# thomasneff/AdaNeRF

Hardware: NVIDIA H100
Metric: frames_per_sec_800x800 (higher is better)
Workload: dtype bf16

## Files before the change

### adanerf_b200/csrc/api.cu

```cuda
#include <cuda_runtime.h>

#include <algorithm>
#include <cmath>
#include <cstdio>
#include <cstdlib>
#include <cstring>
#include <map>
#include <optional>
#include <string>
#include <vector>

#include "../../include/adanerf_b200.h"
#include "export_loader.h"
#include "mlp.cuh"
#include "ptx.cuh"
#include "stages.cuh"

using namespace adn;

namespace {

struct HostTensor {
  std::vector<float> data;
  int64_t rows = 0, cols = 0;
// ... 60 lines not shown
  cudaEvent_t ev[8] = {};
  adn_stats stats{};
  std::string last_error;
};

namespace {

const char* kStatusText[] = {"ok", "invalid argument", "CUDA error", "no usable sm_90 device", "weights not set",
                             "I/O error", "device watchdog tripped"};

adn_status fail(adn_ctx* ctx, adn_status s, const std::string& msg) {
  if (ctx) ctx->last_error = msg;
  return s;
}
adn_status cuda_fail(adn_ctx* ctx, cudaError_t e, const char* where) {
  return fail(ctx, ADN_ERR_CUDA, std::string(where) + ": " + cudaGetErrorString(e));
}
#define ADN_CUDA(ctx, call)                                   \
  do {                                                        \
    cudaError_t e__ = (call);                                 \
    if (e__ != cudaSuccess) return cuda_fail(ctx, e__, #call); \
  } while (0)

adn_status ensure(adn_ctx* ctx, Buf& b, size_t bytes) {
  if (bytes <= b.cap) return ADN_OK;
  ADN_CUDA(ctx, b.release());
  const bool pinned = b.kind == Buf::kPinned;
  const size_t want = pinned ? bytes : bytes + bytes / 8 + 256;
  ADN_CUDA(ctx, pinned ? cudaMallocHost(&b.p, want) : cudaMalloc(&b.p, want));
  b.cap = want;
  return ADN_OK;
}

bool pin_in_place(adn_ctx* ctx, const void* p, size_t bytes) {
  const char* lo = static_cast<const char*>(p);
  for (const adn_ctx::Reg& r : ctx->regs)
    if (lo >= static_cast<const char*>(r.p) && lo + bytes <= static_cast<const char*>(r.p) + r.bytes) return true;
  cudaPointerAttributes attr{};
  if (cudaPointerGetAttributes(&attr, p) == cudaSuccess && attr.type == cudaMemoryTypeHost) return true;
  cudaGetLastError();
  return false;
}

inline uint16_t f2bf(float f) {
  uint32_t u;
  std::memcpy(&u, &f, 4);
  if ((u & 0x7FFFFFFFu) > 0x7F800000u) return uint16_t((u >> 16) | 0x40);
  u += 0x7FFFu + ((u >> 16) & 1u);
  return uint16_t(u >> 16);
}
inline float bf2f(uint16_t h) {
  uint32_t u = uint32_t(h) << 16;
  float f;
  std::memcpy(&f, &u, 4);
  return f;
}

struct Seg {
  int col0, valid;
};

void pack_layer(const float* W, int n_out, int k_in, const std::vector<Seg>& segs, int nsplit, std::vector<uint8_t>& blob) {
  const int n_half = (n_out + 127) / 128;
  for (int nh = 0; nh < n_half; ++nh) {
    for (const Seg& sg : segs) {
      const size_t base = blob.size();
      blob.resize(base + size_t(nsplit) * kBlkBytes, 0);
      for (int n = 0; n < 128; ++n) {
        const int row = nh * 128 + n;
        for (int kk = 0; kk < 64; ++kk) {
          float w = 0.0f;
          if (row < n_out && kk < sg.valid && sg.col0 + kk < k_in) w = W[size_t(row) * k_in + sg.col0 + kk];
          const uint16_t hi = f2bf(w);
          const uint32_t off = sw128_offset(uint32_t(n), uint32_t(kk));
          std::memcpy(&blob[base + off], &hi, 2);
          if (nsplit == 2) {
            const uint16_t lo = f2bf(w - bf2f(hi));
            std::memcpy(&blob[base + kBlkBytes + off], &lo, 2);
          }
        }
      }
    }
  }
}

size_t push_floats(std::vector<float>& f, const float* src, size_t n) {
  while (f.size() % 4) f.push_back(0.0f);
  const size_t off = f.size();
  f.insert(f.end(), src, src + n);
  while (f.size() % 4) f.push_back(0.0f);
  return off;
}

const HostTensor* find(const Net& n, const std::string& name) {
  auto it = n.tensors.find(name);
  return it == n.tensors.end() ? nullptr : &it->second;
}

adn_status upload(adn_ctx* ctx, Net& net, const std::vector<uint8_t>& wblob, const std::vector<float>& fblob) {
  if (fblob.size() > size_t(kSideFloats))
    return fail(ctx, ADN_ERR_INVALID, "network has " + std::to_string(fblob.size()) + " fp32 side parameters (biases and heads), more than " +
                                          std::to_string(kSideFloats) + " fit in shared memory");
  std::memset(net.prog.side, 0, sizeof(net.prog.side));
  std::memcpy(net.prog.side, fblob.data(), fblob.size() * 4);
  adn_status s = ensure(ctx, net.wblob, wblob.size());
  if (s != ADN_OK) return s;
  ADN_CUDA(ctx, cudaMemcpy(net.wblob.p, wblob.data(), wblob.size(), cudaMemcpyHostToDevice));
  return ADN_OK;
}

adn_status build_net0(adn_ctx* ctx) {
  Net& net = ctx->net[0];
  auto bad = [&](const std::string& msg) { return fail(ctx, ADN_ERR_INVALID, "sampling net: " + msg); };
  int D = 0;
  while (find(net, "layers." + std::to_string(D) + ".weight")) ++D;
  if (D < 1 || D > kMaxLayers) return bad("need layers.0.weight .. (1-12 layers)");
  const int nsplit = ctx->mlp0_terms == 3 ? 2 : 1;
  const int width = int(find(net, "layers.0.weight")->rows);
  MlpProgram P{};
  P.n_layers = D;
  std::vector<uint8_t> wblob;
  std::vector<float> fblob;
  int prev = -1;
  for (int l = 0; l < D; ++l) {
    const std::string name = "layers." + std::to_string(l);
    const HostTensor* W = find(net, name + ".weight");
    const HostTensor* B = find(net, name + ".bias");
    if (!B || int64_t(B->data.size()) != W->rows) return bad(name + ".bias is missing or not [" + std::to_string(W->rows) + "]");
    const int n_out = int(W->rows), k_in = int(W->cols);
    const bool last = (l == D - 1);
    if (l == 0) {
      if (k_in < 1 || k_in > 128) return bad(name + ".weight has " + std::to_string(k_in) + " input columns; the input width must be 1-128");
      net.n_in = k_in;
    } else if (k_in != prev) {
      return bad(name + ".weight has " + std::to_string(k_in) + " input columns but layers." + std::to_string(l - 1) + " has " +
                 std::to_string(prev) + " outputs: layer widths must chain (BaseNet skips are not supported)");
    }
    if (!last && n_out != width)
      return bad(name + ".weight has " + std::to_string(n_out) + " outputs; every hidden layer must be as wide as layers.0 (" +
                 std::to_string(width) + ")");
    if (!last && n_out != 128 && n_out != 256)
      return bad(name + ".weight has " + std::to_string(n_out) + " outputs; the hidden width must be 128 or 256");
    if (last && n_out != 128 && n_out != 256)
      return bad(name + ".weight has " + std::to_string(n_out) + " outputs; the output width must be 128 or 256");
    prev = n_out;
    MlpLayer& L = P.layers[l];
    std::vector<Seg> segs;
    if (l == 0) {
      segs = {{0, std::min(64, k_in)}, {64, std::max(0, k_in - 64)}};
    } else {
      for (int c = 0; c < k_in; c += 64) segs.push_back({c, 64});
    }
    L.n_kb = uint8_t(segs.size());
    for (size_t i = 0; i < segs.size(); ++i) {
      L.a_blk[i] = uint8_t(i);
      L.k_cnt[i] = uint8_t(std::max(i == 0 ? 1 : 0, (segs[i].valid + 15) / 16));
    }
    L.n_half = uint8_t(n_out / 128);
    L.flags = last ? uint8_t(LF_FINAL_RAW) : uint8_t(LF_RELU | LF_OUT_ACT);
    L.out_blk0 = 0;
    L.w_off = uint32_t(wblob.size());
    pack_layer(W->data.data(), n_out, k_in, segs, nsplit, wblob);
    L.bias_off = uint32_t(push_floats(fblob, B->data.data(), B->data.size()));
    if (last) {
      net.n_out = n_out;
      P.out_cols = n_out;
    }
  }
  P.in = sampling_tiles(net.n_in, nsplit);
  P.in_nblk0 = P.in.n_blk;
  net.prog = P;
  adn_status s = upload(ctx, net, wblob, fblob);
  if (s != ADN_OK) return s;
  net.depth = D;
  net.width = width;
  net.skip = -1;
  net.ready = true;
  return ADN_OK;
}

adn_status build_net1(adn_ctx* ctx) {
  Net& net = ctx->net[1];
  constexpr int kP = 63, kV = 27;
  auto bad = [&](const std::string& msg) { return fail(ctx, ADN_ERR_INVALID, "shading net: " + msg); };
  auto shape = [](int64_t r, int64_t c) { return "[" + std::to_string(r) + ", " + std::to_string(c) + "]"; };
  const HostTensor* w0 = find(net, "pts_linears.0.weight");
  if (!w0 || w0->cols != kP)
    return bad("pts_linears.0.weight must be [W, 63] (posEnc 10-4)" + (w0 ? ", not " + shape(w0->rows, w0->cols) : std::string(", missing")));
  const int W = int(w0->rows);
  if (W != 128 && W != 256) return bad("pts_linears.0.weight has " + std::to_string(W) + " rows; the width W must be 128 or 256");
  int D = 0;
  while (find(net, "pts_linears." + std::to_string(D) + ".weight")) ++D;
  if (D > kMaxLayers - 2) return bad("pts_linears.0 .. " + std::to_string(D - 1) + ": " + std::to_string(D) + " layers, at most 10 are supported");
  const HostTensor *pw[kMaxLayers], *pb[kMaxLayers];
  int skip = -1;
  for (int i = 0; i < D; ++i) {
    const std::string name = "pts_linears." + std::to_string(i);
    pw[i] = find(net, name + ".weight");
    pb[i] = find(net, name + ".bias");
    if (pw[i]->rows != W) return bad(name + ".weight has " + std::to_string(pw[i]->rows) + " rows; every pts layer must be W = " + std::to_string(W) + " wide");
    if (i > 0 && pw[i]->cols == W + kP) {
      if (skip >= 0)
        return bad(name + ".weight reads cat[pts, h] after the skip at layer " + std::to_string(skip) + "; at most one skip is supported");
      skip = i - 1;
    } else if (i > 0 && pw[i]->cols != W) {
      return bad(name + ".weight has " + std::to_string(pw[i]->cols) + " input columns; expect W = " + std::to_string(W) +
                 " or W + 63 = " + std::to_string(W + kP) + " (a skip)");
    }
    if (!pb[i] || int64_t(pb[i]->data.size()) != W) return bad(name + ".bias is missing or not [" + std::to_string(W) + "]");
  }
  struct Want {
    const char* name;
    int64_t rows, cols;
  };
  const Want want[4] = {{"feature_linear", W, W}, {"alpha_linear", 1, W}, {"views_linears.0", W / 2, W + kV}, {"rgb_linear", 3, W / 2}};
  const HostTensor *hw[4], *hb[4];
  for (int j = 0; j < 4; ++j) {
    const std::string name(want[j].name);
    hw[j] = find(net, name + ".weight");
    hb[j] = find(net, name + ".bias");
    if (!hw[j] || hw[j]->rows != want[j].rows || hw[j]->cols != want[j].cols)
      return bad(name + ".weight must be " + shape(want[j].rows, want[j].cols) + " for W = " + std::to_string(W) + " (posEnc 10-4)" +
                 (hw[j] ? ", not " + shape(hw[j]->rows, hw[j]->cols) : std::string(", missing")));
    if (!hb[j] || int64_t(hb[j]->data.size()) != want[j].rows) return bad(name + ".bias is missing or not [" + std::to_string(want[j].rows) + "]");
  }
  const HostTensor *fw = hw[0], *fb = hb[0], *aw = hw[1], *ab = hb[1], *vw = hw[2], *vb = hb[2], *rw = hw[3], *rb = hb[3];
  net.n_in = kP + kV;
  net.n_out = 4;
  const int nh = W / 64;
  const int load_v = skip >= 0 ? skip + 1 : 0;
  MlpProgram P{};
  P.n_layers = D + 2;
  std::vector<uint8_t> wblob;
  std::vector<float> fblob;
  for (int l = 0; l < D + 2; ++l) {
    MlpLayer& L = P.layers[l];
    std::vector<Seg> segs;
    std::vector<uint8_t> blk;
    auto read_p = [&] { segs.push_back({0, kP}), blk.push_back(0); };
    auto read_hidden = [&](int col0) {
      for (int b = 0; b < nh; ++b) segs.push_back({col0 + 64 * b, 64}), blk.push_back(uint8_t(1 + b));
    };
    const HostTensor *Wt, *B;
    L.out_blk0 = 1;
    L.n_half = uint8_t(W / 128);
    if (l < D) {
      if (l == 0) {
        read_p();
      } else if (l == skip + 1) {
        read_p();
        read_hidden(kP);
      } else {
        read_hidden(0);
      }
      L.flags = LF_RELU | LF_OUT_ACT | (l == D - 1 ? LF_ALPHA_DOT : 0) | (l == load_v ? LF_LOAD_IN1_AFTER : 0);
      Wt = pw[l];
      B = pb[l];
    } else if (l == D) {
      read_hidden(0);
      L.flags = LF_OUT_ACT;
      Wt = fw;
      B = fb;
    } else {
      read_hidden(0);
      segs.push_back({W, kV});
      blk.push_back(0);
      L.flags = LF_RELU | LF_FINAL_RGB | LF_WAIT_IN;
      L.n_half = 1;
      Wt = vw;
      B = vb;
    }
    L.n_kb = uint8_t(segs.size());
    for (size_t i = 0; i < segs.size(); ++i) {
      L.a_blk[i] = blk[i];
      L.k_cnt[i] = uint8_t((segs[i].valid + 15) / 16);
    }
    L.w_off = uint32_t(wblob.size());
    pack_layer(Wt->data.data(), int(Wt->rows), int(Wt->cols), segs, 1, wblob);
    std::vector<float> bias(size_t(L.n_half) * 128, 0.0f);
    std::copy(B->data.begin(), B->data.end(), bias.begin());
    L.bias_off = uint32_t(push_floats(fblob, bias.data(), bias.size()));
  }
  std::vector<float> rgb_w(3 * 128, 0.0f);
  for (int k = 0; k < 3; ++k) std::copy_n(rw->data.data() + size_t(k) * (W / 2), W / 2, rgb_w.data() + k * 128);
  P.alpha_w_off = uint32_t(push_floats(fblob, aw->data.data(), size_t(W)));
  P.alpha_b_off = uint32_t(push_floats(fblob, ab->data.data(), 1));
  P.rgb_w_off = uint32_t(push_floats(fblob, rgb_w.data(), rgb_w.size()));
  P.rgb_b_off = uint32_t(push_floats(fblob, rb->data.data(), 3));
  P.in = shading_tiles();
  P.in_nblk0 = 1;
  P.out_cols = 4;
  net.prog = P;
  adn_status s = upload(ctx, net, wblob, fblob);
  if (s != ADN_OK) return s;
  net.depth = D;
  net.width = W;
  net.skip = skip;
  net.ready = true;
  return ADN_OK;
}

void set_ndc_projection(adn_ctx* ctx, int W, int H, float focal_in) {
  const double focal = focal_in > 0.0f ? double(focal_in) : 0.5 * double(W) / std::tan(0.5 * double(ctx->scene.fov));
  ctx->sc.ndc_cw = float(-1.0 / (double(W) / (2.0 * focal)));
  ctx->sc.ndc_ch = float(-1.0 / (double(H) / (2.0 * focal)));
}

adn_status ensure_dense_lut(adn_ctx* ctx, int K) {
  if (ctx->dense_K == K) return ADN_OK;
  std::vector<float> lut(K);
  const double max_v = double(ctx->scene.depth_range[1]) - double(ctx->scene.depth_range[0]);
  for (int k = 0; k < K; ++k) {
    const float step = 1.0f / float(K);
    const float lin = (k < (K + 1) / 2) ? float(k) * step : 1.0f - float(K - k) * step;
    const float t = lin + float(0.5 / K);
    const float z = ctx->scene.z_near * (1.0f - t) + ctx->scene.z_far * t;
    const float w = float(std::pow(max_v + 1.0, double(z)));
    lut[k] = ctx->scene.use_ndc ? z : (w - 1.0f) + ctx->scene.depth_range[0];
  }
  adn_status s = ensure(ctx, ctx->zlut_dense, sizeof(float) * K);
  if (s != ADN_OK) return s;
  ADN_CUDA(ctx, cudaMemcpy(ctx->zlut_dense.p, lut.data(), sizeof(float) * K, cudaMemcpyHostToDevice));
  ctx->dense_K = K;
  return ADN_OK;
}

PoseDev make_pose(const float* pose, const float* rot) {
  PoseDev p;
  std::memcpy(p.pose, pose, 12);
  std::memcpy(p.rot, rot, 36);
  return p;
}

std::optional<CameraRays> camera_rays(const adn_ctx* ctx, int W, int H, int row0, int rows) {
  if (!ctx || W < 1 || H < 1 || row0 < 0 || rows < 0 || row0 + rows > H) return std::nullopt;
  CameraRays c;
  const double fov = double(ctx->scene.fov);
  const double focal = 0.5 * W / std::tan(0.5 * fov);
  const double x_dist = std::tan(fov / 2) * focal;
  const double y_dist = x_dist * (double(H) / double(W));
  c.x_pp = x_dist / (W / 2.0);
  c.y_pp = y_dist / (H / 2.0);
  c.start_x = -(x_dist - c.x_pp / 2);
  c.start_y = -(y_dist - c.y_pp / 2);
  c.focal = focal;
  c.W = W;
  c.H = H;
  c.row0 = row0;
  return c;
}

int64_t pad128(int64_t n) { return (n + 127) / 128 * 128; }

adn_status run_mlp(adn_ctx* ctx, int id, const uint8_t* tiles, float* out, const long long* rows_dev, long long rows,
                   cudaStream_t st, const EncodeParams* enc = nullptr) {
  Net& n = ctx->net[id];
  const cudaError_t e = launch_mlp(n.prog, n.wblob.as<uint8_t>(), tiles, out, rows_dev, rows, ctx->d_err, ctx->num_sms, st, enc);
  if (e != cudaSuccess) return cuda_fail(ctx, e, id == 0 ? "launch sampling MLP" : "launch shading MLP");
  ctx->stats.kernel_launches++;
  return ADN_OK;
}

struct RenderCall {
  const float* pose;
  const float* rot;
  const float* d_dirs = nullptr;
  std::optional<CameraRays> cam;
  int64_t n_rays;
  float thr;
  int K;
  float* d_rgb = nullptr;
  uint8_t* d_rgba8 = nullptr;
  int32_t* d_nsamples = nullptr;
  float* d_oracle_w = nullptr;
  adn_aux_outputs aux{};
  cudaStream_t st;
  RenderCall(const float* pose_, const float* rot_, int64_t n_rays_, float thr_, int K_, void* stream)
      : pose(pose_), rot(rot_), n_rays(n_rays_), thr(thr_), K(K_), st(static_cast<cudaStream_t>(stream)) {}
};

RenderCall chunk_of(const RenderCall& call, int64_t r0, int64_t chunk) {
  RenderCall c = call;
  c.n_rays = std::min(chunk, call.n_rays - r0);
  if (c.d_dirs) c.d_dirs += 3 * r0;
  if (c.cam) c.cam->row0 += int(r0 / c.cam->W);
  if (c.d_rgb) c.d_rgb += 3 * r0;
  if (c.d_rgba8) c.d_rgba8 += 4 * r0;
  if (c.d_nsamples) c.d_nsamples += r0;
  if (c.d_oracle_w) c.d_oracle_w += 128 * r0;
  for (float** p : {&c.aux.d_weights, &c.aux.d_alpha, &c.aux.d_z_vals})
    if (*p) *p += r0 * c.K;
  for (float** p : {&c.aux.d_depth_map, &c.aux.d_acc_map, &c.aux.d_disp_map, &c.aux.d_depth_est})
    if (*p) *p += r0;
  return c;
}

Stage5Aux stage5_aux(const adn_ctx* ctx, const adn_aux_outputs& a) {
  const adn_scene& sc = ctx->scene;
  return {a.d_weights, a.d_alpha, a.d_z_vals, a.d_depth_map, a.d_acc_map, a.d_disp_map, a.d_depth_est, sc.use_ndc ? 1 : 0,
          sc.depth_range[0], float(std::log(double(sc.depth_range[1]) - double(sc.depth_range[0]) + 1.0))};
}

adn_status run_stages_0_1(adn_ctx* ctx, const RenderCall& c, int64_t w, bool timing) {
  const Net& n0 = ctx->net[0];
  adn_status s = ensure(ctx, ctx->tiles0, size_t(pad128(c.n_rays) / 128) * n0.prog.in.tile_bytes());
  if (s != ADN_OK) return s;
  float* raw0 = c.d_oracle_w ? c.d_oracle_w : ctx->raw0.as<float>() + 128 * w;
  uint8_t* tiles0 = ctx->tiles0.as<uint8_t>();
  if (timing) cudaEventRecord(ctx->ev[0], c.st);
  ADN_CUDA(ctx, launch_stage0(ctx->sc, make_pose(c.pose, c.rot), c.d_dirs, c.cam ? &*c.cam : nullptr, c.n_rays, nullptr,
                              ctx->ray_o.as<float>() + 3 * w, ctx->ray_d.as<float>() + 3 * w, tiles0, n0.prog.in.n_terms, c.st));
  ctx->stats.kernel_launches++;
  if (timing) cudaEventRecord(ctx->ev[1], c.st);
  if ((s = run_mlp(ctx, 0, tiles0, raw0, nullptr, c.n_rays, c.st)) != ADN_OK) return s;
  if (timing) cudaEventRecord(ctx->ev[2], c.st);
  return ADN_OK;
}

adn_status run_stages_2_5(adn_ctx* ctx, const RenderCall& c, int64_t w, const float* d_thr, bool timing) {
  const int64_t n = c.n_rays;
  const int K = c.K;
  const bool dense = (c.thr == 0.0f);
  const int64_t cap = n * K;
  adn_status s;
  if ((s = ensure(ctx, ctx->count, size_t(n) * 4)) != ADN_OK) return s;
  if ((s = ensure(ctx, ctx->offset, size_t(n) * 4)) != ADN_OK) return s;
  if (!dense) {
    if ((s = ensure(ctx, ctx->rayidx, size_t(cap) * 4)) != ADN_OK) return s;
    if ((s = ensure(ctx, ctx->zbuf, size_t(cap) * 4)) != ADN_OK) return s;
// ... 618 lines not shown
```

### adanerf_b200/csrc/mlp.cu

```cuda
#include <cuda_bf16.h>
#include <cuda_runtime.h>

#include "mlp.cuh"
#include "posenc.cuh"
#include "ptx.cuh"
#include "tiles.cuh"

namespace adn {

template <uint8_t V>
struct ConstFlags {
  __device__ constexpr operator uint8_t() const { return V; }
};

template <int NSPLIT>
struct MlpCfg {
  static constexpr int kNB = (NSPLIT == 2) ? 4 : 5;
  static constexpr int kStageBytes = NSPLIT * kBlkBytes;
  static constexpr int kStages = (NSPLIT == 2) ? 2 : 8;
  static constexpr size_t kActBytes = size_t(NSPLIT) * kNB * kBlkBytes;
  static constexpr size_t kSmemBytes =
      kActBytes + size_t(kStages) * kStageBytes + size_t(kSideFloats) * 4 + 2 * kStages * 8 + 1024 ;
};
static_assert(MlpCfg<1>::kSmemBytes <= 232448 && MlpCfg<2>::kSmemBytes <= 232448, "shared memory per block (sm_90)");

template <bool VIEW>
__device__ __forceinline__ void encode_row(const EncodeParams& enc, long long i, long long rows, uint8_t* blk, int row) {
  float f[64];
#pragma unroll
  for (int k = 0; k < 64; ++k) f[k] = 0.0f;
  if (i < rows) {
    long long ray;
    float zw;
    if (enc.ray_idx) {
      ray = enc.ray_idx[i];
      zw = enc.z[i];
    } else {
      ray = i / enc.K;
      zw = enc.zlut_dense[i - ray * enc.K];
    }
    float pos[3], dir[3];
    sample_inputs(enc.sc, false, enc.ray_o, enc.ray_d, ray, zw, pos, dir);
    if (VIEW) posenc3<4>(dir, f);
    else posenc3<10>(pos, f);
  }
#pragma unroll
  for (int ch = 0; ch < 8; ++ch) pack_chunk8(f + ch * 8, uint32_t(row), ch, blk, nullptr);
}

__device__ __forceinline__ void copy_rows(const uint8_t* __restrict__ src, uint32_t dst, int nblk, int wg, int tw) {
  for (int b = 0; b < nblk; ++b) {
    const uint4* s = reinterpret_cast<const uint4*>(src + size_t(b) * kBlkBytes + size_t(wg) * (kBlkBytes / 2));
    const uint32_t d = dst + uint32_t(b) * kBlkBytes + uint32_t(wg) * (kBlkBytes / 2);
    uint4 v[4];
#pragma unroll
    for (int j = 0; j < 4; ++j) v[j] = __ldg(s + tw + 128 * j);
#pragma unroll
    for (int j = 0; j < 4; ++j) st_shared_v4(d + uint32_t(tw + 128 * j) * 16u, v[j].x, v[j].y, v[j].z, v[j].w);
  }
}

template <int NSPLIT, bool ENC>
__global__ void __launch_bounds__(kMlpThreads, 1)
mlp_kernel(const __grid_constant__ MlpProgram prog, const uint8_t* __restrict__ wblob, const uint8_t* __restrict__ in_tiles,
           float* __restrict__ out, const long long* __restrict__ rows_dev, long long rows_host, int* err_flag,
           const __grid_constant__ EncodeParams enc) {
  static_assert(!ENC || NSPLIT == 1, "fused input encoder: shading net (plain bf16) only");
  using Cfg = MlpCfg<NSPLIT>;
  constexpr int NB = Cfg::kNB;
  constexpr int STAGES = Cfg::kStages;
  constexpr int STAGE_BYTES = Cfg::kStageBytes;
  constexpr int kConsumerWarps = 8, kProducerWarp = 8;

  extern __shared__ uint8_t smem_raw[];
  uint8_t* smem = smem_raw + ((1024u - (smem_u32(smem_raw) & 1023u)) & 1023u);
  uint8_t* act = smem;
  uint8_t* ring = act + Cfg::kActBytes;
  float* side = reinterpret_cast<float*>(ring + size_t(STAGES) * STAGE_BYTES);
  uint64_t* w_full = reinterpret_cast<uint64_t*>(side + kSideFloats);
  uint64_t* w_empty = w_full + STAGES;

  const int warp = __shfl_sync(0xffffffffu, int(threadIdx.x >> 5), 0);
  const int lane = threadIdx.x & 31;
  const long long rows = rows_dev ? *rows_dev : rows_host;
  const long long n_tiles = (rows + kTileM - 1) / kTileM;

  for (int i = threadIdx.x; i < kSideFloats; i += blockDim.x) side[i] = prog.side[i];
  if (threadIdx.x == 0) {
    for (int s = 0; s < STAGES; ++s) {
      mbar_init(&w_full[s], 1);
      mbar_init(&w_empty[s], kConsumerWarps);
    }
    mbar_fence_init();
  }
  __syncthreads();

  if (warp >= kProducerWarp) {
    setmaxnreg_dec<40>();
    if (warp == kProducerWarp && lane == 0) {
      int stage = 0;
      uint32_t phase = 0;
      for (long long t = blockIdx.x; t < n_tiles; t += gridDim.x) {
        for (int l = 0; l < prog.n_layers; ++l) {
          const MlpLayer& L = prog.layers[l];
          const int n_st = int(L.n_kb) * int(L.n_half);
          for (int i = 0; i < n_st; ++i) {
            mbar_wait(&w_empty[stage], phase ^ 1, err_flag, 1);
            mbar_arrive_expect_tx(&w_full[stage], STAGE_BYTES);
            bulk_g2s(ring + size_t(stage) * STAGE_BYTES, wblob + L.w_off + size_t(i) * STAGE_BYTES, STAGE_BYTES, &w_full[stage]);
            if (++stage == STAGES) {
              stage = 0;
              phase ^= 1;
            }
          }
        }
      }
    }
    return;
  }

  setmaxnreg_inc<232>();
  const int wg = warp >> 2;
  const int tw = threadIdx.x & 127;
  const int r0 = 64 * wg + 16 * (warp & 3) + (lane >> 2);
  const int cq = 2 * (lane & 3);
  const int bar_id = 1 + wg;
  const uint32_t act_s = smem_u32(act);
  const uint32_t ring_s = smem_u32(ring);
  const uint32_t wg_off = uint32_t(wg) * (kBlkBytes / 2);
  auto blk_addr = [&](int term, int blk) -> uint32_t { return act_s + uint32_t(term * NB + blk) * kBlkBytes; };
  const uint64_t desc_hi = make_desc_sw128(0) & ~uint64_t(0x3FFF);
  auto desc = [&](uint32_t addr) -> uint64_t { return desc_hi | uint64_t((addr & 0x3FFFF) >> 4); };

  int stage = 0;
  uint32_t phase = 0;
  for (long long t = blockIdx.x; t < n_tiles; t += gridDim.x) {
    if (ENC) {
      if (tw < 64) encode_row<false>(enc, t * kTileM + 64 * wg + tw, rows, act, 64 * wg + tw);
    } else {
#pragma unroll
      for (int term = 0; term < NSPLIT; ++term)
        copy_rows(in_tiles + size_t(t) * prog.in.tile_bytes() + prog.in.blk_off(term, 0), blk_addr(term, 0), prog.in_nblk0, wg, tw);
    }
    fence_proxy_async_smem();
    named_bar_sync(bar_id, 128);
    float alpha[2] = {0.0f, 0.0f};
    for (int l = 0; l < prog.n_layers; ++l) {
      const MlpLayer& L = prog.layers[l];
      float acc[2][64];
      int prev = -1;
#pragma unroll
      for (int nh = 0; nh < 2; ++nh) {
        if (nh >= L.n_half) break;
        for (int kb = 0; kb < L.n_kb; ++kb) {
          const uint32_t a_hi = blk_addr(0, L.a_blk[kb]) + wg_off;
          const uint32_t a_lo = a_hi + uint32_t(NSPLIT - 1) * NB * kBlkBytes;
          const uint32_t b_hi = ring_s + uint32_t(stage) * STAGE_BYTES;
          const uint32_t b_lo = b_hi + uint32_t(NSPLIT - 1) * kBlkBytes;
          const int nk = L.k_cnt[kb];
          mbar_wait(&w_full[stage], phase, err_flag, 2);
          wgmma_fence();
#pragma unroll
          for (int k = 0; k < 4; ++k) {
            if (k < nk) {
              wgmma_m64n128_bf16(acc[nh], desc(a_hi + 32 * k), desc(b_hi + 32 * k), (kb > 0 || k > 0) ? 1u : 0u);
              if (NSPLIT == 2) {
                wgmma_m64n128_bf16(acc[nh], desc(a_lo + 32 * k), desc(b_hi + 32 * k), 1u);
                wgmma_m64n128_bf16(acc[nh], desc(a_hi + 32 * k), desc(b_lo + 32 * k), 1u);
              }
            }
          }
          wgmma_commit();
          wgmma_wait<1>();
          if (prev >= 0 && lane == 0) mbar_arrive(&w_empty[prev]);
          prev = stage;
          if (++stage == STAGES) {
            stage = 0;
            phase ^= 1;
          }
        }
      }
      wgmma_wait<0>();
      if (lane == 0) mbar_arrive(&w_empty[prev]);
      named_bar_sync(bar_id, 128);

      auto epilogue = [&](auto flags) {
        float rgb[2][3] = {{0.f, 0.f, 0.f}, {0.f, 0.f, 0.f}};
#pragma unroll
        for (int nh = 0; nh < 2; ++nh) {
          if (nh >= L.n_half) break;
#pragma unroll
          for (int i = 0; i < 16; ++i) {
            const int col = nh * 128 + 8 * i + cq;
            const float2 b = *reinterpret_cast<const float2*>(side + L.bias_off + col);
#pragma unroll
            for (int rr = 0; rr < 2; ++rr) {
              const int row = r0 + 8 * rr;
              float v0 = acc[nh][4 * i + 2 * rr] + b.x;
              float v1 = acc[nh][4 * i + 2 * rr + 1] + b.y;
              if (flags & LF_FINAL_RAW) {
                const long long grow = t * kTileM + row;
                if (grow < rows) *reinterpret_cast<float2*>(out + grow * prog.out_cols + col) = make_float2(v0, v1);
                continue;
              }
              if (flags & LF_RELU) {
                v0 = fmaxf(v0, 0.0f);
                v1 = fmaxf(v1, 0.0f);
              }
              if (flags & LF_ALPHA_DOT) {
                const float2 w = *reinterpret_cast<const float2*>(side + prog.alpha_w_off + col);
                alpha[rr] = fmaf(v1, w.y, fmaf(v0, w.x, alpha[rr]));
              }
              if (flags & LF_OUT_ACT) {
                const uint32_t off = uint32_t(L.out_blk0 + (col >> 6)) * kBlkBytes + sw128_offset(uint32_t(row), uint32_t(col & 63));
                const uint32_t hi = bf16x2(v0, v1);
                *reinterpret_cast<uint32_t*>(act + off) = hi;
                if (NSPLIT == 2) *reinterpret_cast<uint32_t*>(act + NB * kBlkBytes + off) = bf16x2_lo(v0, v1, hi);
              }
              if (flags & LF_FINAL_RGB) {
#pragma unroll
                for (int k = 0; k < 3; ++k) {
                  const float2 w = *reinterpret_cast<const float2*>(side + prog.rgb_w_off + k * 128 + col);
                  rgb[rr][k] = fmaf(v1, w.y, fmaf(v0, w.x, rgb[rr][k]));
                }
              }
            }
          }
        }
        if (flags & LF_FINAL_RGB) {
#pragma unroll
          for (int rr = 0; rr < 2; ++rr) {
            float a = alpha[rr], c0 = rgb[rr][0], c1 = rgb[rr][1], c2 = rgb[rr][2];
#pragma unroll
            for (int m = 1; m <= 2; m <<= 1) {
              a += __shfl_xor_sync(0xffffffffu, a, m);
              c0 += __shfl_xor_sync(0xffffffffu, c0, m);
              c1 += __shfl_xor_sync(0xffffffffu, c1, m);
              c2 += __shfl_xor_sync(0xffffffffu, c2, m);
            }
            const long long grow = t * kTileM + r0 + 8 * rr;
            if ((lane & 3) == 0 && grow < rows)
              reinterpret_cast<float4*>(out)[grow] = make_float4(c0 + side[prog.rgb_b_off], c1 + side[prog.rgb_b_off + 1],
                                                                 c2 + side[prog.rgb_b_off + 2], a + side[prog.alpha_b_off]);
          }
        }
      };
      using F = uint8_t;
      constexpr F kEpiFlags = LF_RELU | LF_ALPHA_DOT | LF_OUT_ACT | LF_FINAL_RAW | LF_FINAL_RGB;
      switch (L.flags & kEpiFlags) {
        case LF_RELU | LF_OUT_ACT: epilogue(ConstFlags<LF_RELU | LF_OUT_ACT>{}); break;
        case LF_RELU | LF_OUT_ACT | LF_ALPHA_DOT: epilogue(ConstFlags<LF_RELU | LF_OUT_ACT | LF_ALPHA_DOT>{}); break;
        case LF_OUT_ACT: epilogue(ConstFlags<LF_OUT_ACT>{}); break;
        case LF_RELU | LF_FINAL_RGB: epilogue(ConstFlags<LF_RELU | LF_FINAL_RGB>{}); break;
        case LF_FINAL_RAW: epilogue(ConstFlags<LF_FINAL_RAW>{}); break;
        default: epilogue(F(L.flags)); break;
      }
      if (L.flags & LF_LOAD_IN1_AFTER) {
        if (ENC) {
          if (tw < 64) encode_row<true>(enc, t * kTileM + 64 * wg + tw, rows, act, 64 * wg + tw);
        } else {
          copy_rows(in_tiles + size_t(t) * prog.in.tile_bytes() + prog.in.blk_off(0, prog.in_nblk0), blk_addr(0, 0), 1, wg, tw);
        }
      }
      fence_proxy_async_smem();
      named_bar_sync(bar_id, 128);
    }
  }
}

__global__ void pack_rows_kernel(const float* __restrict__ x, long long rows_host, const long long* __restrict__ rows_dev,
                                 int n_feat, const __grid_constant__ TileFormat fmt, uint8_t* __restrict__ tiles) {
  const long long rows = rows_dev ? *rows_dev : rows_host;
  const long long n_tiles = (rows + kTileM - 1) / kTileM;
  const long long total = n_tiles * kTileM * fmt.n_blk * 8;
  for (long long i = blockIdx.x * (long long)blockDim.x + threadIdx.x; i < total; i += (long long)gridDim.x * blockDim.x) {
    const int chunk = int(i & 7);
    const long long rb = i >> 3;
    const int blk = int(rb % fmt.n_blk);
    const long long row = rb / fmt.n_blk;
    const long long t = row >> 7;
    pack_tile_chunk(fmt, tiles + size_t(t) * fmt.tile_bytes(), blk, uint32_t(row & (kTileM - 1)), chunk,
                    [&](int c) { return row < rows ? x[row * n_feat + c] : 0.0f; });
  }
}

cudaError_t set_max_dyn_smem_once(const void* func, int bytes, unsigned long long* done) {
  int dev = 0;
  cudaError_t e = cudaGetDevice(&dev);
  if (e != cudaSuccess) return e;
  if (dev < 64 && ((__atomic_load_n(done, __ATOMIC_ACQUIRE) >> dev) & 1ull)) return cudaSuccess;
  e = cudaFuncSetAttribute(func, cudaFuncAttributeMaxDynamicSharedMemorySize, bytes);
  if (e != cudaSuccess) return e;
  if (dev < 64) __atomic_fetch_or(done, 1ull << dev, __ATOMIC_RELEASE);
  return cudaSuccess;
}

template <int NSPLIT, bool ENC>
static cudaError_t launch_mlp_t(const MlpProgram& prog, const uint8_t* wblob, const uint8_t* in_tiles, float* out,
                                const long long* rows_dev, long long rows_host, int* err_flag, int num_sms, cudaStream_t stream,
                                const EncodeParams& enc) {
  static unsigned long long attr_done = 0;
  const size_t smem = MlpCfg<NSPLIT>::kSmemBytes;
  auto kernel = mlp_kernel<NSPLIT, ENC>;
  cudaError_t e = set_max_dyn_smem_once(reinterpret_cast<const void*>(kernel), int(smem), &attr_done);
  if (e != cudaSuccess) return e;
  long long grid = num_sms;
  if (!rows_dev) {
    const long long n_tiles = (rows_host + kTileM - 1) / kTileM;
    if (n_tiles < grid) grid = n_tiles < 1 ? 1 : n_tiles;
  }
  kernel<<<unsigned(grid), kMlpThreads, smem, stream>>>(prog, wblob, in_tiles, out, rows_dev, rows_host, err_flag, enc);
  return cudaGetLastError();
}

cudaError_t launch_mlp(const MlpProgram& prog, const uint8_t* wblob, const uint8_t* in_tiles, float* out,
                       const long long* rows_dev, long long rows_host, int* err_flag, int num_sms, cudaStream_t stream,
                       const EncodeParams* enc) {
  if (enc) {
    if (prog.in.n_terms != 1) return cudaErrorInvalidValue;
    return launch_mlp_t<1, true>(prog, wblob, in_tiles, out, rows_dev, rows_host, err_flag, num_sms, stream, *enc);
  }
  if (prog.in.n_terms == 2) return launch_mlp_t<2, false>(prog, wblob, in_tiles, out, rows_dev, rows_host, err_flag, num_sms, stream, EncodeParams{});
  return launch_mlp_t<1, false>(prog, wblob, in_tiles, out, rows_dev, rows_host, err_flag, num_sms, stream, EncodeParams{});
}

cudaError_t launch_pack_rows(const float* x, long long rows, const long long* rows_dev, int n_feat, const TileFormat& fmt,
                             uint8_t* tiles, int num_sms, cudaStream_t stream) {
  long long work = ((rows + kTileM - 1) / kTileM) * kTileM * fmt.n_blk * 8;
  int grid = int((work + 255) / 256);
  if (grid < 1) grid = 1;
  if (grid > 16 * num_sms) grid = 16 * num_sms;
  pack_rows_kernel<<<grid, 256, 0, stream>>>(x, rows, rows_dev, n_feat, fmt, tiles);
  return cudaGetLastError();
}

}
```

### adanerf_b200/csrc/mlp.cuh

```cuda
#pragma once
#include <cstdint>
#include <cuda_runtime.h>

#include "stages.cuh"
#include "tiles.cuh"

namespace adn {

constexpr int kMaxLayers = 12;
constexpr int kMlpThreads = 384;
constexpr int kSideFloats = 3592;

enum : uint8_t {
  LF_RELU = 1,
  LF_ALPHA_DOT = 2,
  LF_OUT_ACT = 4,
  LF_FINAL_RAW = 8,
  LF_FINAL_RGB = 16,
  LF_LOAD_IN1_AFTER = 32,
  LF_WAIT_IN = 64
};

struct MlpLayer {
  uint32_t w_off;
  uint32_t bias_off;
  uint8_t n_kb;
  uint8_t a_blk[6];
  uint8_t n_half;
  uint8_t flags;
  uint8_t out_blk0;
  uint8_t k_cnt[6];
};

struct MlpProgram {
  int32_t n_layers;
  TileFormat in;
  int32_t in_nblk0;
  uint32_t alpha_w_off, alpha_b_off, rgb_w_off, rgb_b_off;
  int32_t out_cols;
  MlpLayer layers[kMaxLayers];
  float side[kSideFloats];
};

struct EncodeParams {
  const float* ray_o = nullptr;
  const float* ray_d = nullptr;
  const int32_t* ray_idx = nullptr;
  const float* z = nullptr;
  const float* zlut_dense = nullptr;
  int K = 1;
  SceneDev sc{};
};

cudaError_t set_max_dyn_smem_once(const void* func, int bytes, unsigned long long* done);

cudaError_t launch_mlp(const MlpProgram& prog, const uint8_t* wblob, const uint8_t* in_tiles, float* out,
                       const long long* rows_dev, long long rows_host, int* err_flag, int num_sms, cudaStream_t stream,
                       const EncodeParams* enc = nullptr);
cudaError_t launch_pack_rows(const float* x, long long rows, const long long* rows_dev, int n_feat, const TileFormat& fmt,
                             uint8_t* tiles, int num_sms, cudaStream_t stream);

}
```

### adanerf_b200/csrc/ptx.cuh

```cuda
#pragma once
#include <cstdint>
#include <cuda_runtime.h>

namespace adn {

__device__ __forceinline__ uint32_t smem_u32(const void* p) {
  return static_cast<uint32_t>(__cvta_generic_to_shared(p));
}

__device__ __forceinline__ bool elect_one() {
  uint32_t pred;
  asm volatile("{\n\t.reg .pred p;\n\telect.sync _|p, 0xffffffff;\n\tselp.b32 %0, 1, 0, p;\n\t}" : "=r"(pred));
  return pred != 0;
}

__device__ __forceinline__ void st_shared_v4(uint32_t addr, uint32_t x, uint32_t y, uint32_t z, uint32_t w) {
  asm volatile("st.shared.v4.b32 [%0], {%1, %2, %3, %4};" ::"r"(addr), "r"(x), "r"(y), "r"(z), "r"(w) : "memory");
}

__device__ __forceinline__ float4 ld_shared_f4(uint32_t addr) {
  float4 v;
  asm volatile("ld.shared.v4.f32 {%0, %1, %2, %3}, [%4];" : "=f"(v.x), "=f"(v.y), "=f"(v.z), "=f"(v.w) : "r"(addr));
  return v;
}

__device__ __forceinline__ void named_bar_sync(int id, int nthreads) {
  asm volatile("bar.sync %0, %1;" ::"r"(id), "r"(nthreads) : "memory");
}
__device__ __forceinline__ void named_bar_arrive(int id, int nthreads) {
  asm volatile("bar.arrive %0, %1;" ::"r"(id), "r"(nthreads) : "memory");
}

__device__ __forceinline__ void mbar_init(uint64_t* bar, uint32_t count) {
  asm volatile("mbarrier.init.shared::cta.b64 [%0], %1;" ::"r"(smem_u32(bar)), "r"(count) : "memory");
}
__device__ __forceinline__ void mbar_fence_init() {
  asm volatile("fence.mbarrier_init.release.cluster;" ::: "memory");
}
__device__ __forceinline__ void mbar_arrive(uint64_t* bar) {
  asm volatile("{\n\t.reg .b64 st;\n\tmbarrier.arrive.shared::cta.b64 st, [%0];\n\t}" ::"r"(smem_u32(bar)) : "memory");
}
__device__ __forceinline__ void mbar_arrive_expect_tx(uint64_t* bar, uint32_t bytes) {
  asm volatile("{\n\t.reg .b64 st;\n\tmbarrier.arrive.expect_tx.shared::cta.b64 st, [%0], %1;\n\t}" ::"r"(smem_u32(bar)),
               "r"(bytes)
               : "memory");
}
__device__ __forceinline__ bool mbar_try_wait(uint64_t* bar, uint32_t parity) {
  uint32_t ok;
  asm volatile(
      "{\n\t.reg .pred p;\n\t"
      "mbarrier.try_wait.parity.shared::cta.b64 p, [%1], %2, %3;\n\t"
      "selp.b32 %0, 1, 0, p;\n\t}"
      : "=r"(ok)
      : "r"(smem_u32(bar)), "r"(parity), "r"(0x989680u)
      : "memory");
  return ok != 0;
}

#ifndef ADN_WATCHDOG_CYCLES
#define ADN_WATCHDOG_CYCLES (4000000000ll)
#endif
static __device__ __forceinline__ void mbar_wait_slow(uint64_t* bar, uint32_t parity, int* err_flag, int site) {
  const long long t0 = clock64();
  while (!mbar_try_wait(bar, parity)) {
    if (clock64() - t0 > ADN_WATCHDOG_CYCLES) {
      if (err_flag) atomicExch(err_flag, 0x1000 + site);
      __threadfence_system();
      asm volatile("trap;");
    }
  }
}
__device__ __forceinline__ void mbar_wait(uint64_t* bar, uint32_t parity, int* err_flag, int site) {
  if (mbar_try_wait(bar, parity)) return;
  mbar_wait_slow(bar, parity, err_flag, site);
}

__device__ __forceinline__ void bulk_g2s(void* smem_dst, const void* gmem_src, uint32_t bytes, uint64_t* bar) {
  asm volatile("cp.async.bulk.shared::cluster.global.mbarrier::complete_tx::bytes [%0], [%1], %2, [%3];" ::"r"(
                   smem_u32(smem_dst)),
               "l"(gmem_src), "r"(bytes), "r"(smem_u32(bar))
               : "memory");
}
__device__ __forceinline__ void bulk_s2g(void* gmem_dst, const void* smem_src, uint32_t bytes) {
  asm volatile("cp.async.bulk.global.shared::cta.bulk_group [%0], [%1], %2;" ::"l"(gmem_dst), "r"(smem_u32(smem_src)), "r"(bytes)
               : "memory");
}
__device__ __forceinline__ void bulk_commit() { asm volatile("cp.async.bulk.commit_group;" ::: "memory"); }
__device__ __forceinline__ void bulk_wait_read_all() { asm volatile("cp.async.bulk.wait_group.read 0;" ::: "memory"); }
__device__ __forceinline__ void bulk_wait_all() { asm volatile("cp.async.bulk.wait_group 0;" ::: "memory"); }

__device__ __forceinline__ void fence_proxy_async_all() { asm volatile("fence.proxy.async;" ::: "memory"); }
__device__ __forceinline__ void fence_proxy_async_smem() {
  asm volatile("fence.proxy.async.shared::cta;" ::: "memory");
}

template <int N>
__device__ __forceinline__ void setmaxnreg_inc() { asm volatile("setmaxnreg.inc.sync.aligned.u32 %0;" ::"n"(N)); }
template <int N>
__device__ __forceinline__ void setmaxnreg_dec() { asm volatile("setmaxnreg.dec.sync.aligned.u32 %0;" ::"n"(N)); }

__device__ __forceinline__ void wgmma_fence() { asm volatile("wgmma.fence.sync.aligned;" ::: "memory"); }
__device__ __forceinline__ void wgmma_commit() { asm volatile("wgmma.commit_group.sync.aligned;" ::: "memory"); }
template <int N>
__device__ __forceinline__ void wgmma_wait() { asm volatile("wgmma.wait_group.sync.aligned %0;" ::"n"(N) : "memory"); }

__device__ __forceinline__ void wgmma_m64n128_bf16(float (&d)[64], uint64_t a_desc, uint64_t b_desc, uint32_t accumulate) {
  asm volatile(
      "{\n\t.reg .pred p;\n\tsetp.ne.b32 p, %66, 0;\n\t"
      "wgmma.mma_async.sync.aligned.m64n128k16.f32.bf16.bf16 "
      "{%0, %1, %2, %3, %4, %5, %6, %7, %8, %9, %10, %11, %12, %13, %14, %15, "
      "%16, %17, %18, %19, %20, %21, %22, %23, %24, %25, %26, %27, %28, %29, %30, %31, "
      "%32, %33, %34, %35, %36, %37, %38, %39, %40, %41, %42, %43, %44, %45, %46, %47, "
      "%48, %49, %50, %51, %52, %53, %54, %55, %56, %57, %58, %59, %60, %61, %62, %63}, "
      "%64, %65, p, 1, 1, 0, 0;\n\t}"
      : "+f"(d[0]), "+f"(d[1]), "+f"(d[2]), "+f"(d[3]), "+f"(d[4]), "+f"(d[5]), "+f"(d[6]), "+f"(d[7]), "+f"(d[8]),
        "+f"(d[9]), "+f"(d[10]), "+f"(d[11]), "+f"(d[12]), "+f"(d[13]), "+f"(d[14]), "+f"(d[15]), "+f"(d[16]),
        "+f"(d[17]), "+f"(d[18]), "+f"(d[19]), "+f"(d[20]), "+f"(d[21]), "+f"(d[22]), "+f"(d[23]), "+f"(d[24]),
        "+f"(d[25]), "+f"(d[26]), "+f"(d[27]), "+f"(d[28]), "+f"(d[29]), "+f"(d[30]), "+f"(d[31]), "+f"(d[32]),
        "+f"(d[33]), "+f"(d[34]), "+f"(d[35]), "+f"(d[36]), "+f"(d[37]), "+f"(d[38]), "+f"(d[39]), "+f"(d[40]),
        "+f"(d[41]), "+f"(d[42]), "+f"(d[43]), "+f"(d[44]), "+f"(d[45]), "+f"(d[46]), "+f"(d[47]), "+f"(d[48]),
        "+f"(d[49]), "+f"(d[50]), "+f"(d[51]), "+f"(d[52]), "+f"(d[53]), "+f"(d[54]), "+f"(d[55]), "+f"(d[56]),
        "+f"(d[57]), "+f"(d[58]), "+f"(d[59]), "+f"(d[60]), "+f"(d[61]), "+f"(d[62]), "+f"(d[63])
      : "l"(a_desc), "l"(b_desc), "r"(accumulate)
      : "memory");
}

__device__ __forceinline__ uint64_t make_desc_sw128(uint32_t smem_addr_bytes) {
  uint64_t d = 0;
  d |= static_cast<uint64_t>((smem_addr_bytes & 0x3FFFF) >> 4);
  d |= static_cast<uint64_t>(1) << 16;
  d |= static_cast<uint64_t>(1024 >> 4) << 32;
  d |= static_cast<uint64_t>(1) << 62;
  return d;
}

__host__ __device__ __forceinline__ uint32_t sw128_offset(uint32_t row, uint32_t col) {
  const uint32_t chunk = (col >> 3) ^ (row & 7);
  return (row >> 3) * 1024u + (row & 7) * 128u + chunk * 16u + (col & 7) * 2u;
}

}
```

Measured before the change: 51.19.

## Keep hidden activations in registers and feed WGMMA from register A operands

```diff
diff --git a/adanerf_b200/csrc/api.cu b/adanerf_b200/csrc/api.cu
--- a/adanerf_b200/csrc/api.cu
+++ b/adanerf_b200/csrc/api.cu
@@ -236,13 +236,12 @@
       for (int c = 0; c < k_in; c += 64) segs.push_back({c, 64});
     }
     L.n_kb = uint8_t(segs.size());
+    (l == 0 ? L.in_first : L.n_hid) = L.n_kb;
     for (size_t i = 0; i < segs.size(); ++i) {
-      L.a_blk[i] = uint8_t(i);
       L.k_cnt[i] = uint8_t(std::max(i == 0 ? 1 : 0, (segs[i].valid + 15) / 16));
     }
     L.n_half = uint8_t(n_out / 128);
     L.flags = last ? uint8_t(LF_FINAL_RAW) : uint8_t(LF_RELU | LF_OUT_ACT);
-    L.out_blk0 = 0;
     L.w_off = uint32_t(wblob.size());
     pack_layer(W->data.data(), n_out, k_in, segs, nsplit, wblob);
     L.bias_off = uint32_t(push_floats(fblob, B->data.data(), B->data.size()));
@@ -320,13 +319,12 @@
   for (int l = 0; l < D + 2; ++l) {
     MlpLayer& L = P.layers[l];
     std::vector<Seg> segs;
-    std::vector<uint8_t> blk;
-    auto read_p = [&] { segs.push_back({0, kP}), blk.push_back(0); };
+    auto read_p = [&] { segs.push_back({0, kP}), L.in_first = 1; };
     auto read_hidden = [&](int col0) {
-      for (int b = 0; b < nh; ++b) segs.push_back({col0 + 64 * b, 64}), blk.push_back(uint8_t(1 + b));
+      for (int b = 0; b < nh; ++b) segs.push_back({col0 + 64 * b, 64});
+      L.n_hid = uint8_t(nh);
     };
     const HostTensor *Wt, *B;
-    L.out_blk0 = 1;
     L.n_half = uint8_t(W / 128);
     if (l < D) {
       if (l == 0) {
@@ -348,17 +346,14 @@
     } else {
       read_hidden(0);
       segs.push_back({W, kV});
-      blk.push_back(0);
-      L.flags = LF_RELU | LF_FINAL_RGB | LF_WAIT_IN;
+      L.in_last = 1;
+      L.flags = LF_RELU | LF_FINAL_RGB;
       L.n_half = 1;
       Wt = vw;
       B = vb;
     }
     L.n_kb = uint8_t(segs.size());
-    for (size_t i = 0; i < segs.size(); ++i) {
-      L.a_blk[i] = blk[i];
-      L.k_cnt[i] = uint8_t((segs[i].valid + 15) / 16);
-    }
+    for (size_t i = 0; i < segs.size(); ++i) L.k_cnt[i] = uint8_t((segs[i].valid + 15) / 16);
     L.w_off = uint32_t(wblob.size());
     pack_layer(Wt->data.data(), int(Wt->rows), int(Wt->cols), segs, 1, wblob);
     std::vector<float> bias(size_t(L.n_half) * 128, 0.0f);
diff --git a/adanerf_b200/csrc/mlp.cu b/adanerf_b200/csrc/mlp.cu
--- a/adanerf_b200/csrc/mlp.cu
+++ b/adanerf_b200/csrc/mlp.cu
@@ -15,7 +15,7 @@
 
 template <int NSPLIT>
 struct MlpCfg {
-  static constexpr int kNB = (NSPLIT == 2) ? 4 : 5;
+  static constexpr int kNB = (NSPLIT == 2) ? 4 : 2;
   static constexpr int kStageBytes = NSPLIT * kBlkBytes;
   static constexpr int kStages = (NSPLIT == 2) ? 2 : 8;
   static constexpr size_t kActBytes = size_t(NSPLIT) * kNB * kBlkBytes;
@@ -96,7 +96,7 @@
   __syncthreads();
 
   if (warp >= kProducerWarp) {
-    setmaxnreg_dec<40>();
+    setmaxnreg_dec<24>();
     if (warp == kProducerWarp && lane == 0) {
       int stage = 0;
       uint32_t phase = 0;
@@ -119,7 +119,7 @@
     return;
   }
 
-  setmaxnreg_inc<232>();
+  setmaxnreg_inc<240>();
   const int wg = warp >> 2;
   const int tw = threadIdx.x & 127;
   const int r0 = 64 * wg + 16 * (warp & 3) + (lane >> 2);
@@ -132,8 +132,38 @@
   const uint64_t desc_hi = make_desc_sw128(0) & ~uint64_t(0x3FFF);
   auto desc = [&](uint32_t addr) -> uint64_t { return desc_hi | uint64_t((addr & 0x3FFFF) >> 4); };
 
+  uint32_t afrag[4][4][4];
+  auto clear_afrag = [&](int kb0, int kb1) {
+#pragma unroll
+    for (int kb = 0; kb < 4; ++kb)
+#pragma unroll
+      for (int k = 0; k < 4; ++k)
+#pragma unroll
+        for (int j = 0; j < 4; ++j)
+          if (kb >= kb0 && kb < kb1) afrag[kb][k][j] = 0u;
+  };
+
   int stage = 0;
   uint32_t phase = 0;
+  int prev = -1;
+  auto k_block = [&](bool first, int nk, auto mma) {
+    mbar_wait(&w_full[stage], phase, err_flag, 2);
+    wgmma_fence();
+    const uint32_t b = ring_s + uint32_t(stage) * STAGE_BYTES;
+#pragma unroll
+    for (int k = 0; k < 4; ++k) {
+      if (k < nk) mma(k, b, (first && k == 0) ? 0u : 1u);
+    }
+    wgmma_commit();
+    wgmma_wait<1>();
+    if (prev >= 0 && lane == 0) mbar_arrive(&w_empty[prev]);
+    prev = stage;
+    if (++stage == STAGES) {
+      stage = 0;
+      phase ^= 1;
+    }
+  };
+
   for (long long t = blockIdx.x; t < n_tiles; t += gridDim.x) {
     if (ENC) {
       if (tw < 64) encode_row<false>(enc, t * kTileM + 64 * wg + tw, rows, act, 64 * wg + tw);
@@ -144,51 +174,62 @@
     }
     fence_proxy_async_smem();
     named_bar_sync(bar_id, 128);
+    if (NSPLIT == 1) clear_afrag(0, 4);
     float alpha[2] = {0.0f, 0.0f};
     for (int l = 0; l < prog.n_layers; ++l) {
       const MlpLayer& L = prog.layers[l];
       float acc[2][64];
-      int prev = -1;
 #pragma unroll
       for (int nh = 0; nh < 2; ++nh) {
         if (nh >= L.n_half) break;
-        for (int kb = 0; kb < L.n_kb; ++kb) {
-          const uint32_t a_hi = blk_addr(0, L.a_blk[kb]) + wg_off;
-          const uint32_t a_lo = a_hi + uint32_t(NSPLIT - 1) * NB * kBlkBytes;
-          const uint32_t b_hi = ring_s + uint32_t(stage) * STAGE_BYTES;
-          const uint32_t b_lo = b_hi + uint32_t(NSPLIT - 1) * kBlkBytes;
-          const int nk = L.k_cnt[kb];
-          mbar_wait(&w_full[stage], phase, err_flag, 2);
-          wgmma_fence();
-#pragma unroll
-          for (int k = 0; k < 4; ++k) {
-            if (k < nk) {
-              wgmma_m64n128_bf16(acc[nh], desc(a_hi + 32 * k), desc(b_hi + 32 * k), (kb > 0 || k > 0) ? 1u : 0u);
-              if (NSPLIT == 2) {
-                wgmma_m64n128_bf16(acc[nh], desc(a_lo + 32 * k), desc(b_hi + 32 * k), 1u);
-                wgmma_m64n128_bf16(acc[nh], desc(a_hi + 32 * k), desc(b_lo + 32 * k), 1u);
-              }
-            }
-          }
-          wgmma_commit();
-          wgmma_wait<1>();
-          if (prev >= 0 && lane == 0) mbar_arrive(&w_empty[prev]);
-          prev = stage;
-          if (++stage == STAGES) {
-            stage = 0;
-            phase ^= 1;
-          }
+        if (NSPLIT == 2) {
+          for (int kb = 0; kb < L.n_kb; ++kb) {
+            const uint32_t a_hi = blk_addr(0, kb) + wg_off;
+            const uint32_t a_lo = a_hi + uint32_t(NB) * kBlkBytes;
+            k_block(kb == 0, L.k_cnt[kb], [&](int k, uint32_t b_hi, uint32_t accumulate) {
+              const uint32_t b_lo = b_hi + uint32_t(kBlkBytes);
+              wgmma_m64n128_bf16(acc[nh], desc(a_hi + 32 * k), desc(b_hi + 32 * k), accumulate);
+              wgmma_m64n128_bf16(acc[nh], desc(a_lo + 32 * k), desc(b_hi + 32 * k), 1u);
+              wgmma_m64n128_bf16(acc[nh], desc(a_hi + 32 * k), desc(b_lo + 32 * k), 1u);
+            });
+          }
+        } else {
+          auto from_smem = [&](int blk) {
+            const uint32_t a = blk_addr(0, blk) + wg_off;
+            return [&, a](int k, uint32_t b, uint32_t accumulate) {
+              wgmma_m64n128_bf16(acc[nh], desc(a + 32 * k), desc(b + 32 * k), accumulate);
+            };
+          };
+#pragma unroll
+          for (int ib = 0; ib < NB; ++ib) {
+            if (ib >= L.in_first) break;
+            k_block(ib == 0, L.k_cnt[ib], from_smem(ib));
+          }
+#pragma unroll
+          for (int hb = 0; hb < 4; ++hb) {
+            if (hb >= L.n_hid) break;
+            k_block(hb == 0 && L.in_first == 0, 4, [&](int k, uint32_t b, uint32_t accumulate) {
+              wgmma_m64n128_bf16_rs(acc[nh], afrag[hb][k], desc(b + 32 * k), accumulate);
+            });
+          }
+          if (L.in_last) k_block(L.n_kb == 1, L.k_cnt[L.n_kb - 1], from_smem(0));
         }
       }
       wgmma_wait<0>();
       if (lane == 0) mbar_arrive(&w_empty[prev]);
-      named_bar_sync(bar_id, 128);
+      prev = -1;
+      const bool input_next = (L.flags & LF_LOAD_IN1_AFTER) || l + 1 == prog.n_layers;
+      if (NSPLIT == 2 || input_next) named_bar_sync(bar_id, 128);
 
       auto epilogue = [&](auto flags) {
         float rgb[2][3] = {{0.f, 0.f, 0.f}, {0.f, 0.f, 0.f}};
+        if (NSPLIT == 1 && !(flags & LF_OUT_ACT)) clear_afrag(0, 4);
 #pragma unroll
         for (int nh = 0; nh < 2; ++nh) {
-          if (nh >= L.n_half) break;
+          if (nh >= L.n_half) {
+            if (NSPLIT == 1 && (flags & LF_OUT_ACT)) clear_afrag(2 * nh, 4);
+            break;
+          }
 #pragma unroll
           for (int i = 0; i < 16; ++i) {
             const int col = nh * 128 + 8 * i + cq;
@@ -212,10 +253,14 @@
                 alpha[rr] = fmaf(v1, w.y, fmaf(v0, w.x, alpha[rr]));
               }
               if (flags & LF_OUT_ACT) {
-                const uint32_t off = uint32_t(L.out_blk0 + (col >> 6)) * kBlkBytes + sw128_offset(uint32_t(row), uint32_t(col & 63));
                 const uint32_t hi = bf16x2(v0, v1);
-                *reinterpret_cast<uint32_t*>(act + off) = hi;
-                if (NSPLIT == 2) *reinterpret_cast<uint32_t*>(act + NB * kBlkBytes + off) = bf16x2_lo(v0, v1, hi);
+                if (NSPLIT == 1) {
+                  afrag[2 * nh + (i >> 3)][(i >> 1) & 3][2 * (i & 1) + rr] = hi;
+                } else {
+                  const uint32_t off = uint32_t(col >> 6) * kBlkBytes + sw128_offset(uint32_t(row), uint32_t(col & 63));
+                  *reinterpret_cast<uint32_t*>(act + off) = hi;
+                  *reinterpret_cast<uint32_t*>(act + NB * kBlkBytes + off) = bf16x2_lo(v0, v1, hi);
+                }
               }
               if (flags & LF_FINAL_RGB) {
 #pragma unroll
@@ -262,8 +307,10 @@
           copy_rows(in_tiles + size_t(t) * prog.in.tile_bytes() + prog.in.blk_off(0, prog.in_nblk0), blk_addr(0, 0), 1, wg, tw);
         }
       }
-      fence_proxy_async_smem();
-      named_bar_sync(bar_id, 128);
+      if (NSPLIT == 2 || (L.flags & LF_LOAD_IN1_AFTER)) {
+        fence_proxy_async_smem();
+        named_bar_sync(bar_id, 128);
+      }
     }
   }
 }
diff --git a/adanerf_b200/csrc/mlp.cuh b/adanerf_b200/csrc/mlp.cuh
--- a/adanerf_b200/csrc/mlp.cuh
+++ b/adanerf_b200/csrc/mlp.cuh
@@ -17,18 +17,16 @@
   LF_OUT_ACT = 4,
   LF_FINAL_RAW = 8,
   LF_FINAL_RGB = 16,
-  LF_LOAD_IN1_AFTER = 32,
-  LF_WAIT_IN = 64
+  LF_LOAD_IN1_AFTER = 32
 };
 
 struct MlpLayer {
   uint32_t w_off;
   uint32_t bias_off;
   uint8_t n_kb;
-  uint8_t a_blk[6];
+  uint8_t in_first, n_hid, in_last;
   uint8_t n_half;
   uint8_t flags;
-  uint8_t out_blk0;
   uint8_t k_cnt[6];
 };
 
diff --git a/adanerf_b200/csrc/ptx.cuh b/adanerf_b200/csrc/ptx.cuh
--- a/adanerf_b200/csrc/ptx.cuh
+++ b/adanerf_b200/csrc/ptx.cuh
@@ -125,6 +125,27 @@
       : "memory");
 }
 
+__device__ __forceinline__ void wgmma_m64n128_bf16_rs(float (&d)[64], const uint32_t (&a)[4], uint64_t b_desc, uint32_t accumulate) {
+  asm volatile(
+      "{\n\t.reg .pred p;\n\tsetp.ne.b32 p, %69, 0;\n\t"
+      "wgmma.mma_async.sync.aligned.m64n128k16.f32.bf16.bf16 "
+      "{%0, %1, %2, %3, %4, %5, %6, %7, %8, %9, %10, %11, %12, %13, %14, %15, "
+      "%16, %17, %18, %19, %20, %21, %22, %23, %24, %25, %26, %27, %28, %29, %30, %31, "
+      "%32, %33, %34, %35, %36, %37, %38, %39, %40, %41, %42, %43, %44, %45, %46, %47, "
+      "%48, %49, %50, %51, %52, %53, %54, %55, %56, %57, %58, %59, %60, %61, %62, %63}, "
+      "{%64, %65, %66, %67}, %68, p, 1, 1, 0;\n\t}"
+      : "+f"(d[0]), "+f"(d[1]), "+f"(d[2]), "+f"(d[3]), "+f"(d[4]), "+f"(d[5]), "+f"(d[6]), "+f"(d[7]), "+f"(d[8]),
+        "+f"(d[9]), "+f"(d[10]), "+f"(d[11]), "+f"(d[12]), "+f"(d[13]), "+f"(d[14]), "+f"(d[15]), "+f"(d[16]),
+        "+f"(d[17]), "+f"(d[18]), "+f"(d[19]), "+f"(d[20]), "+f"(d[21]), "+f"(d[22]), "+f"(d[23]), "+f"(d[24]),
+        "+f"(d[25]), "+f"(d[26]), "+f"(d[27]), "+f"(d[28]), "+f"(d[29]), "+f"(d[30]), "+f"(d[31]), "+f"(d[32]),
+        "+f"(d[33]), "+f"(d[34]), "+f"(d[35]), "+f"(d[36]), "+f"(d[37]), "+f"(d[38]), "+f"(d[39]), "+f"(d[40]),
+        "+f"(d[41]), "+f"(d[42]), "+f"(d[43]), "+f"(d[44]), "+f"(d[45]), "+f"(d[46]), "+f"(d[47]), "+f"(d[48]),
+        "+f"(d[49]), "+f"(d[50]), "+f"(d[51]), "+f"(d[52]), "+f"(d[53]), "+f"(d[54]), "+f"(d[55]), "+f"(d[56]),
+        "+f"(d[57]), "+f"(d[58]), "+f"(d[59]), "+f"(d[60]), "+f"(d[61]), "+f"(d[62]), "+f"(d[63])
+      : "r"(a[0]), "r"(a[1]), "r"(a[2]), "r"(a[3]), "l"(b_desc), "r"(accumulate)
+      : "memory");
+}
+
 __device__ __forceinline__ uint64_t make_desc_sw128(uint32_t smem_addr_bytes) {
   uint64_t d = 0;
   d |= static_cast<uint64_t>((smem_addr_bytes & 0x3FFFF) >> 4);
```

New measurement: 58.31 (median of 6 runs). 13.9% higher.
